# roljon/Steered-Mixture-of-Experts

Hardware: NVIDIA B200
Metric: pixel_kernel_evals_per_s_fwd_bwd (higher is better)
Workload: dtype f32

## Files before the change

### steered-mixture-of-experts_b200/csrc/forward.cu

```cuda
#include "smoe_common.cuh"
#include "fwd_records.cuh"

namespace smoe {

template <int D, int C>
__device__ __forceinline__ void parabola(const float* __restrict__ f, const float (&xs)[3], float& c, float& b) {
    using R = Rec<D, C>;
    c = f[R::OC];
#pragma unroll
    for (int l = 1; l < D; ++l) {
        float t = f[R::OL + l];
#pragma unroll
        for (int m = l; m < D; ++m) t = fmaf(f[R::OQ + ut(D, l, m)], xs[m], t);
        c = fmaf(t, xs[l], c);
    }
    b = f[R::OL + 0];
#pragma unroll
    for (int m = 1; m < D; ++m) b = fmaf(f[R::OQ + ut(D, 0, m)], xs[m], b);
}

struct FwdArgs {
    smoe_cfg cfg;
    smoe_batch b;
    const float* packed;
    const int32_t* indices;
    const int32_t* counts;
    const float* chunk_bounds;
    const float* lossw;
    const float* ax[3];
    float* rbuf;
    int32_t* argmax;
    uint8_t* infl;
    float* pix;
    float* tile_qmin;
    unsigned long long* pair_counts;
    int ntiles, nt1, nt2, max_chunks;
    float tau, ltau;
    float eps_cut;
};

#ifndef SMOE_FWD_UNROLL
#define SMOE_FWD_UNROLL 2
#endif
constexpr int kBodyUnroll = SMOE_FWD_UNROLL;
template <int D, int C, bool COUNT, bool AMAX>
__global__ void __launch_bounds__(kThreadsF, (D == 2) ? SMOE_FWD_CTAS_2D : 4) forward_kernel(const FwdArgs a) {
    using R = Rec<D, C>;
    constexpr int PK = pstride(D, C);
    constexpr int PPT = kPixPerThread;
    static_assert(kChunk == kThreadsF, "one kernel of a chunk per thread");
    extern __shared__ __align__(128) unsigned char smem_raw[];
    float* raw0 = reinterpret_cast<float*>(smem_raw);
    float* raw1 = raw0 + kChunk * PK;
    float* crec = raw1 + kChunk * PK;
    uint64_t* bar = reinterpret_cast<uint64_t*>(crec + kChunk * R::RC);
    float* red = reinterpret_cast<float*>(bar + 2);
    int* scratch = reinterpret_cast<int*>(red + 32);
    int* clist = scratch + 8;

    const int tid = threadIdx.x;
    const int K = a.counts[0];
    const int nchunks = (K + kChunk - 1) / kChunk;
    const int mode = a.cfg.dense_exec;
    const bool cull = mode == 0, skip = mode != 1;
    if (tid == 0) {
        mbar_init(&bar[0], 1);
        mbar_init(&bar[1], 1);
        fence_barrier_init();
    }
    __syncthreads();
    uint32_t phase0 = 0, phase1 = 0;
    int par = 0;
    unsigned cntA_vis = 0, cntA_ex = 0, cntB_vis = 0, cntB_ex = 0;

    auto issue = [&](int ci, int buf) {
        int nk = min(kChunk, K - ci * kChunk);
        uint32_t bytes = (uint32_t)nk * PK * 4u;
        fence_proxy_async();
        mbar_expect_tx(&bar[buf], bytes);
        tma_load_1d(buf ? raw1 : raw0, a.packed + (size_t)ci * kChunk * PK, bytes, &bar[buf]);
    };

    const int e1 = a.b.tile[1], e2 = a.b.tile[2];
    for (int tile = blockIdx.x; tile < a.ntiles; tile += gridDim.x) {
        int tt[3];
        tt[2] = tile % a.nt2;
        tt[1] = (tile / a.nt2) % a.nt1;
        tt[0] = tile / (a.nt2 * a.nt1);
        int lo[3], hi[3];
        float ctr[3], half[3];
#pragma unroll
        for (int i = 0; i < 3; ++i) {
            lo[i] = a.b.origin[i] + tt[i] * a.b.tile[i];
            hi[i] = min(lo[i] + a.b.tile[i], a.b.origin[i] + a.b.extent[i]) - 1;
            const float c0 = (i < D) ? a.ax[i][lo[i]] : 0.f, c1 = (i < D) ? a.ax[i][hi[i]] : 0.f;
            ctr[i] = 0.5f * (c0 + c1);
            half[i] = 0.5f * (c1 - c0) * 1.0001f + 1e-7f;
        }
        float x0[PPT], xs[3] = {0.f, 0.f, 0.f};
        unsigned okmask = 0;
        const int gbase12 = ((tid / e2) % e1 + lo[1]) * a.b.dims[2] + (tid % e2 + lo[2]);
        unsigned hmask = 0;
        {
            const int i2 = tid % e2, i1 = (tid / e2) % e1;
            const int g1 = lo[1] + i1, g2 = lo[2] + i2;
            auto in_halo = [&](int ax, int g) {
                const int o = a.b.origin[ax], e = o + a.b.extent[ax];
                return ax < D && ((o > 0 && g < o + a.b.halo) || (e < a.b.dims[ax] && g >= e - a.b.halo));
            };
            const bool h12 = a.b.halo > 0 && (in_halo(1, g1) || in_halo(2, g2));
            if (D > 1) xs[1] = a.ax[1][min(g1, hi[1])] - ctr[1];
            if (D > 2) xs[2] = a.ax[2][min(g2, hi[2])] - ctr[2];
#pragma unroll
            for (int p = 0; p < PPT; ++p) {
                const int j = p * kThreadsF + tid;
                const int i0 = j / (e2 * e1);
                const int g0 = lo[0] + i0;
                const bool ok = g0 <= hi[0] && g1 <= hi[1] && g2 <= hi[2];
                bool fed = ok;
                if (a.lossw && ok && a.lossw[g0 * a.b.dims[1] * a.b.dims[2] + gbase12] == SMOE_PIXEL_ABSENT) fed = false;
                if (fed) okmask |= 1u << p;
                if (a.b.halo > 0 && (h12 || in_halo(0, g0))) hmask |= 1u << p;
                x0[p] = a.ax[0][min(g0, hi[0])] - ctr[0];
            }
        }

        auto build_chunk_list = [&](float thr, int part) -> int {
            int n = 0;
            for (int base = 0; base < nchunks; base += kThreadsF) {
                const int ci = base + tid;
                bool need = false;
                if (ci < nchunks) {
                    const float* cb = a.chunk_bounds + (size_t)ci * kCB;
                    float d2 = 0.f, kd = 0.f;
#pragma unroll
                    for (int l = 0; l < D; ++l) {
                        const float mn = cb[l] - ctr[l], mx = cb[3 + l] - ctr[l];
                        const float gap = fmaxf(fmaxf(mn - half[l], -half[l] - mx), 0.f);
                        d2 = fmaf(gap, gap, d2);
                        kd = fmaxf(kd, cb[8 + l] * gap * gap);
                    }
                    const float lam = cb[6], drop = fmaxf(lam * d2, kd);
                    need = part != 1 || !(lam >= 0.f) || !(drop > kNearCut);
                    if (cull && need) need = !(lam >= 0.f) || !(cb[7] - drop < thr);
                }
                int tot;
                const int pos = cta_compact(need, scratch, par, &tot);
                if (need) clist[n + pos] = ci;
                n += tot;
            }
            __syncthreads();
            return n;
        };

        auto sweep = [&](int nlist, float thr, int part, auto&& body) {
            if (tid == 0 && nlist > 0) {
                issue(clist[0], 0);
                if (nlist > 1) issue(clist[1], 1);
            }
            for (int li = 0; li < nlist; ++li) {
                const int buf = li & 1;
                const int ci = clist[li];
                const int nk = min(kChunk, K - ci * kChunk);
                if (buf) { mbar_wait(&bar[1], phase1); phase1 ^= 1; } else { mbar_wait(&bar[0], phase0); phase0 ^= 1; }
                const float* raw = (buf ? raw1 : raw0) + tid * PK;
                bool need = tid < nk;
                float mu[D];
#pragma unroll
                for (int l = 0; l < D; ++l) mu[l] = need ? raw[off_mu(D, C) + l] - ctr[l] : 0.f;
                if (need && (cull || part != 0)) {
                    float d2 = 0.f, kd = 0.f;
#pragma unroll
                    for (int l = 0; l < D; ++l) {
                        const float gap = fmaxf(fabsf(mu[l]) - half[l], 0.f);
                        d2 = fmaf(gap, gap, d2);
                        kd = fmaxf(kd, raw[nparam(D, C) + 1 + l] * gap * gap);
                    }
                    const float lam = raw[nparam(D, C)], drop = fmaxf(lam * d2, kd);
                    if (part != 0) need = (part == 1) == (!(lam >= 0.f) || !(drop > kNearCut));
                    if (need && cull) need = !(lam >= 0.f) || !(raw[off_pi(D, C)] - drop < thr);
                }
                int nneed;
                const int pos = cta_compact(need, scratch, par, &nneed);
                if (need) transform_record<D, C>(raw, mu, ctr, a.indices[ci * kChunk + tid], crec + pos * R::RC);
                __syncthreads();
                if (tid == 0 && li + 2 < nlist) issue(clist[li + 2], buf);
#pragma unroll kBodyUnroll
                for (int kk = 0; kk < nneed; ++kk) body(crec + kk * R::RC);
            }
            __syncthreads();
        };

        float S[PPT];
        float cutA = -126.5f;
        if (a.eps_cut > 0.f && a.tile_qmin) {
            const float Lprev = a.tile_qmin[tile];
            cutA = fmaxf(cutA, Lprev - 2.0f - a.eps_cut);
            if (!(cutA == cutA)) cutA = -126.5f;
        }
        float Lneed = cutA > -126.5f ? cutA + a.eps_cut : -INFINITY;
        for (int attempt = 0; attempt < 2; ++attempt) {
#pragma unroll
            for (int p = 0; p < PPT; ++p) S[p] = 0.f;
            float skipA = cutA + 0.5f;
            auto bodyA = [&](const float* rec) {
                float f[4 * R::NG4];
                const float4* r4 = reinterpret_cast<const float4*>(rec);
#pragma unroll
                for (int j = 0; j < R::NG4; ++j) {
                    float4 v = r4[j];
                    f[4 * j] = v.x; f[4 * j + 1] = v.y; f[4 * j + 2] = v.z; f[4 * j + 3] = v.w;
                }
                float cq, bq;
                parabola<D, C>(f, xs, cq, bq);
                float q[PPT];
                float qmax = -INFINITY;
#pragma unroll
                for (int p = 0; p < PPT; ++p) {
                    q[p] = fmaf(fmaf(f[R::OQ], x0[p], bq), x0[p], cq);
                    qmax = fmaxf(qmax, q[p]);
                }
                if (COUNT) cntA_vis += PPT;
                if (__builtin_expect(!skip || __any_sync(0xffffffffu, qmax >= skipA), 0)) {
#pragma unroll
                    for (int p = 0; p < PPT; ++p) S[p] += ex2f(q[p]);
                    if (COUNT) cntA_ex += PPT;
                }
            };
            sweep(build_chunk_list(cutA, 1), cutA, 1, bodyA);
            {
                float Lt = INFINITY;
#pragma unroll
                for (int p = 0; p < PPT; ++p)
                    if ((okmask >> p) & 1u) Lt = fminf(Lt, log2f(S[p]));
                float Lmin = Lt;
#pragma unroll
                for (int o = 16; o > 0; o >>= 1) Lmin = fminf(Lmin, __shfl_xor_sync(0xffffffffu, Lmin, o));
                if ((tid & 31) == 0) red[tid >> 5] = Lmin;
                __syncthreads();
                Lmin = fminf(fminf(red[0], red[1]), fminf(red[2], red[3]));
                __syncthreads();
                float cut2 = cutA;
                if (skip && Lmin == Lmin) {
                    cut2 = fmaxf(cutA, Lmin - 25.5f);
                    if (Lt == Lt) skipA = fmaxf(skipA, Lt - 25.25f);
                }
                sweep(build_chunk_list(cut2, 2), cut2, 2, bodyA);
            }
            if (!(Lneed > -INFINITY)) break;
            float smin = INFINITY;
#pragma unroll
            for (int p = 0; p < PPT; ++p)
                if ((okmask >> p) & 1u) smin = fminf(smin, log2f(fmaxf(S[p], kSFloor)));
            const int bad = __syncthreads_or(smin < Lneed);
            if (!bad) break;
            cutA = -126.5f;
            Lneed = -INFINITY;
        }

        float qthr[PPT], r[PPT][C], bestw[PPT];
        int bestk[PPT];
        float qmin = INFINITY;
        unsigned live_mask = 0;
#pragma unroll
        for (int p = 0; p < PPT; ++p) {
            if (S[p] > kSFloor) live_mask |= 1u << p;
            float Sc = fmaxf(S[p], kSFloor);
            qthr[p] = ((okmask >> p) & 1u) ? log2f(Sc) : INFINITY;
            qmin = fminf(qmin, qthr[p]);
            bestw[p] = 0.f;
            bestk[p] = -1;
#pragma unroll
            for (int c = 0; c < C; ++c) r[p][c] = 0.f;
        }
#pragma unroll
        for (int o = 16; o > 0; o >>= 1) qmin = fminf(qmin, __shfl_xor_sync(0xffffffffu, qmin, o));
        if ((tid & 31) == 0) red[tid >> 5] = qmin;
        __syncthreads();
        qmin = fminf(fminf(red[0], red[1]), fminf(red[2], red[3]));
        __syncthreads();
        if (tid == 0 && a.tile_qmin) a.tile_qmin[tile] = qmin;
        {
            const float ltau = a.ltau;
            const float thrB = qmin + ltau - 0.01f;
            const int nlist = build_chunk_list(thrB, 0);
            sweep(nlist, thrB, 0, [&](const float* rec) {
                float f[R::RC];
                const float4* r4 = reinterpret_cast<const float4*>(rec);
#pragma unroll
                for (int j = 0; j < R::NG4; ++j) {
                    float4 v = r4[j];
                    f[4 * j] = v.x; f[4 * j + 1] = v.y; f[4 * j + 2] = v.z; f[4 * j + 3] = v.w;
                }
                float cq, bq;
                parabola<D, C>(f, xs, cq, bq);
                float q[PPT];
                bool any = false;
#pragma unroll
                for (int p = 0; p < PPT; ++p) {
                    q[p] = fmaf(fmaf(f[R::OQ], x0[p], bq), x0[p], cq) - qthr[p];
                    any |= (q[p] > ltau);
                }
                if (COUNT) cntB_vis += PPT;
                if (__builtin_expect(!skip || __any_sync(0xffffffffu, any), 0)) {
                    if (COUNT) cntB_ex += PPT;
#pragma unroll
                    for (int j = R::NG4; j < (R::OK + 4) / 4; ++j) {
                        float4 v = r4[j];
                        f[4 * j] = v.x; f[4 * j + 1] = v.y; f[4 * j + 2] = v.z; f[4 * j + 3] = v.w;
                    }
                    const int korig = __float_as_int(f[R::OK]);
                    float Eb[C];
#pragma unroll
                    for (int c = 0; c < C; ++c) {
                        Eb[c] = f[R::ONU + c];
#pragma unroll
                        for (int l = 1; l < D; ++l) Eb[c] = fmaf(f[R::OGA + l * C + c], xs[l], Eb[c]);
                    }
#pragma unroll
                    for (int p = 0; p < PPT; ++p) {
                        const float w = ex2f(q[p]);
                        const bool pass = q[p] > ltau;
                        const float wm = pass ? w : 0.f;
#pragma unroll
                        for (int c = 0; c < C; ++c) r[p][c] = fmaf(wm, fmaf(f[R::OGA + c], x0[p], Eb[c]), r[p][c]);
                        if (AMAX && pass && (w > bestw[p] || (w == bestw[p] && korig < bestk[p]))) { bestw[p] = w; bestk[p] = korig; }
                    }
                    if (any && a.infl) a.infl[korig] = 1;
                }
            });
        }

#pragma unroll
        for (int p = 0; p < PPT; ++p) {
            const int j = p * kThreadsF + tid;
            const bool inb = (okmask >> p) & 1u;
            const int gpix = (lo[0] + j / (e2 * e1)) * a.b.dims[1] * a.b.dims[2] + gbase12;
            const bool halo = ((hmask >> p) & 1u) || (a.lossw && inb && a.lossw[gpix] == SMOE_PIXEL_HALO);
            if (inb && !halo) {
#pragma unroll
                for (int c = 0; c < C; ++c) a.rbuf[(size_t)gpix * C + c] = r[p][c];
                if (AMAX) a.argmax[gpix] = bestk[p];
            }
            if (a.pix) {
                const int RLf = a.b.tile[D - 1];
                float* tp = a.pix + (size_t)tile * pix_stride(D, C, RLf);
                tp[PL_Z * SMOE_TPIX + j] = D == 1 ? x0[p] : xs[D - 1];
                tp[PL_QTHR * SMOE_TPIX + j] = inb ? qthr[p] : INFINITY;
                tp[PL_GR * SMOE_TPIX + j] = (inb && ((live_mask >> p) & 1u)) ? 1.f : 0.f;
                if (D > 1 && j % RLf == 0) {
                    const int row = j / RLf, nrows = SMOE_TPIX / RLf;
                    tp[pix_rowc_offset(C) + row] = x0[p];
#pragma unroll
                    for (int l = 1; l < D - 1; ++l) tp[pix_rowc_offset(C) + l * nrows + row] = xs[l];
                }
            }
        }
    }

    if (COUNT) {
        unsigned long long v[4] = {cntA_vis, cntA_ex, cntB_vis, cntB_ex};
#pragma unroll
        for (int q = 0; q < 4; ++q) {
#pragma unroll
            for (int o = 16; o > 0; o >>= 1) v[q] += __shfl_down_sync(0xffffffffu, v[q], o);
            if ((tid & 31) == 0) atomicAdd(&a.pair_counts[q], v[q]);
        }
    }

}

struct LossArgs {
    smoe_cfg cfg;
    smoe_batch b;
    const float* rbuf;
    const float* image;
    const uint8_t* image_u8;
    const float* lossw;
    float* res;
    float* pix;
    float* scalars;
    float* partials;
    int32_t* ticket;
    int ntiles, nt1, nt2, pix_tstride;
    float eps, q_scale, q_inv_scale;
};

template <int C>
__global__ void __launch_bounds__(256) loss_kernel(const LossArgs a) {
    const int tid = threadIdx.x;
    const int e1 = a.b.tile[1], e2 = a.b.tile[2];
    const int D = a.cfg.d;
    float lsum[C];
#pragma unroll
    for (int c = 0; c < C; ++c) lsum[c] = 0.f;
    float sqsum = 0.f;
    int nonfinite = 0;
    {
        int tt[3], lo[3], hi[3];
        tt[0] = blockIdx.y;
        tt[1] = a.nt2 == 1 ? (int)blockIdx.x : (int)blockIdx.x / a.nt2;
        tt[2] = a.nt2 == 1 ? 0 : (int)blockIdx.x % a.nt2;
        const int tile = (tt[0] * a.nt1 + tt[1]) * a.nt2 + tt[2];
#pragma unroll
        for (int i = 0; i < 3; ++i) {
            lo[i] = a.b.origin[i] + tt[i] * a.b.tile[i];
            hi[i] = min(lo[i] + a.b.tile[i], a.b.origin[i] + a.b.extent[i]) - 1;
        }
        auto in_halo = [&](int ax, int g) {
            const int o = a.b.origin[ax], e = o + a.b.extent[ax];
            return ax < D && ((o > 0 && g < o + a.b.halo) || (e < a.b.dims[ax] && g >= e - a.b.halo));
        };
        float* tp = a.pix ? a.pix + (size_t)tile * a.pix_tstride : nullptr;
        const int i2 = tid % e2, i1 = (tid / e2) % e1;
        const int g1 = lo[1] + i1, g2 = lo[2] + i2;
        const bool in12 = g1 <= hi[1] && g2 <= hi[2];
        const bool halo12 = a.b.halo > 0 && (in_halo(1, g1) || in_halo(2, g2));
        const int rows_per_pass = 256 / (e1 * e2);
        int g0 = lo[0] + tid / (e1 * e2);
        for (int j = tid; j < SMOE_TPIX; j += 256, g0 += rows_per_pass) {
            bool inb = in12 && g0 <= hi[0];
            const int gpix = inb ? (g0 * a.b.dims[1] + g1) * a.b.dims[2] + g2 : 0;
            const float lwv = (a.lossw && inb) ? a.lossw[gpix] : 1.f;
            if (lwv == SMOE_PIXEL_ABSENT) inb = false;
            const bool halo = lwv == SMOE_PIXEL_HALO || halo12 || (a.b.halo > 0 && in_halo(0, g0));
            float g[C], gr = 0.f;
#pragma unroll
            for (int c = 0; c < C; ++c) g[c] = 0.f;
            if (inb && !halo) {
#pragma unroll
                for (int c = 0; c < C; ++c) {
                    const size_t gi = (size_t)gpix * C + c;
                    const float rv = a.rbuf[gi];
                    if (!(fabsf(rv) <= 3.0e38f)) nonfinite = 1;
                    const float rc = fminf(fmaxf(rv, 0.f), 1.f);
                    const float kq = floorf(__fadd_rn(__fmul_rn(rc, a.q_inv_scale), 0.5f));
                    const float rq = __fmul_rn(kq, a.q_scale);
                    const float tgt = a.image_u8 ? __fdiv_rn((float)a.image_u8[gi], 255.0f) : a.image[gi];
                    const float diff = __fsub_rn(rq, tgt);
                    const float ad = fabsf(diff) - a.eps;
                    sqsum = fmaf(diff, diff, sqsum);
                    lsum[c] = a.lossw ? fmaf(ad * ad, lwv, lsum[c]) : fmaf(ad, ad, lsum[c]);
                    const float cw = a.cfg.use_yuv ? (c == 0 ? 0.75f : 0.125f) : (1.0f / C);
                    const float sgn = diff > 0.f ? 1.f : (diff < 0.f ? -1.f : 0.f);
                    const bool ste = (rv >= 0.f) && (rv <= 1.f);
                    g[c] = ste ? 2.f * ad * sgn * cw * a.b.inv_count : 0.f;
                    if (a.lossw) g[c] *= lwv;
                    gr = fmaf(g[c], rv, gr);
                    if (a.res) a.res[gi] = rq;
                }
            }
            if (tp) {
                const bool live = tp[PL_GR * SMOE_TPIX + j] != 0.f;
                tp[PL_GR * SMOE_TPIX + j] = live ? gr : 0.f;
#pragma unroll
                for (int c = 0; c < C; ++c) tp[(PL_G + c) * SMOE_TPIX + j] = g[c];
            }
        }
    }
    __shared__ float red[8][8];
    __shared__ float tree[256];
    __shared__ int s_last;
    const int nblk = gridDim.x * gridDim.y, bid = blockIdx.y * gridDim.x + blockIdx.x;
    float vals[8];
#pragma unroll
    for (int q = 0; q < 8; ++q) vals[q] = 0.f;
#pragma unroll
    for (int c = 0; c < C; ++c) vals[c] = lsum[c];
    vals[4] = sqsum;
    vals[5] = (float)nonfinite;
#pragma unroll
    for (int q = 0; q < 6; ++q)
#pragma unroll
        for (int o = 16; o > 0; o >>= 1) vals[q] += __shfl_down_sync(0xffffffffu, vals[q], o);
    if ((tid & 31) == 0)
#pragma unroll
        for (int q = 0; q < 8; ++q) red[tid >> 5][q] = vals[q];
    __syncthreads();
    if (tid < 8) {
        float s = 0.f;
        for (int wv = 0; wv < 8; ++wv) s += red[wv][tid];
        a.partials[(size_t)bid * 8 + tid] = s;
    }
    __threadfence();
    __syncthreads();
    if (tid == 0) s_last = (atomicAdd(a.ticket, 1) == nblk - 1);
    __syncthreads();
    if (s_last) {
        __threadfence();
        for (int q = 0; q < 6; ++q) {
            float s = 0.f;
            for (int bq = tid; bq < nblk; bq += 256) s += __ldcg(&a.partials[(size_t)bq * 8 + q]);
            tree[tid] = s;
            __syncthreads();
            for (int o = 128; o > 0; o >>= 1) {
                if (tid < o) tree[tid] += tree[tid + o];
                __syncthreads();
            }
            if (tid == 0) a.scalars[q] += tree[0];
            __syncthreads();
        }
        if (tid == 0) *a.ticket = 0;
    }
}

struct CotArgs {
    smoe_batch b;
    const float* rbuf;
    const float* grad_r;
    float* pix;
    int nt1, nt2, pix_tstride;
};

template <int C>
__global__ void __launch_bounds__(256) cotangent_kernel(const CotArgs a) {
    const int tid = threadIdx.x;
    const int e1 = a.b.tile[1], e2 = a.b.tile[2];
    int tt[3], lo[3], hi[3];
    tt[0] = blockIdx.y;
    tt[1] = a.nt2 == 1 ? (int)blockIdx.x : (int)blockIdx.x / a.nt2;
    tt[2] = a.nt2 == 1 ? 0 : (int)blockIdx.x % a.nt2;
    const int tile = (tt[0] * a.nt1 + tt[1]) * a.nt2 + tt[2];
#pragma unroll
    for (int i = 0; i < 3; ++i) {
        lo[i] = a.b.origin[i] + tt[i] * a.b.tile[i];
        hi[i] = min(lo[i] + a.b.tile[i], a.b.origin[i] + a.b.extent[i]) - 1;
    }
    float* tp = a.pix + (size_t)tile * a.pix_tstride;
    const int i2 = tid % e2, i1 = (tid / e2) % e1;
    const int g1 = lo[1] + i1, g2 = lo[2] + i2;
    const bool in12 = g1 <= hi[1] && g2 <= hi[2];
    const int rows_per_pass = 256 / (e1 * e2);
    int g0 = lo[0] + tid / (e1 * e2);
    for (int j = tid; j < SMOE_TPIX; j += 256, g0 += rows_per_pass) {
        const bool inb = in12 && g0 <= hi[0];
        const int gpix = inb ? (g0 * a.b.dims[1] + g1) * a.b.dims[2] + g2 : 0;
        float g[C], gr = 0.f;
#pragma unroll
        for (int c = 0; c < C; ++c) g[c] = 0.f;
        if (inb) {
#pragma unroll
            for (int c = 0; c < C; ++c) {
                const size_t gi = (size_t)gpix * C + c;
                g[c] = a.grad_r[gi];
                gr = fmaf(g[c], a.rbuf[gi], gr);
            }
        }
        const bool live = tp[PL_GR * SMOE_TPIX + j] != 0.f;
        tp[PL_GR * SMOE_TPIX + j] = live ? gr : 0.f;
#pragma unroll
        for (int c = 0; c < C; ++c) tp[(PL_G + c) * SMOE_TPIX + j] = g[c];
    }
}

template <int D, int C>
static size_t fwd_smem_bytes(int max_chunks) {
    return (size_t)(2 * kChunk * pstride(D, C) + kChunk * Rec<D, C>::RC) * 4 + 2 * 8 + 32 * 4 + 8 * 4 +
           (size_t)max_chunks * 4 + 64;
}

}

using namespace smoe;

extern "C" int smoe_forward(const smoe_cfg* cfg, const smoe_batch* batch, const float* packed, const int32_t* indices,
                            const int32_t* counts, const float* chunk_bounds, int K_cap, const float* loss_weights,
                            const float* ax0, const float* ax1, const float* ax2, float* rbuf, int32_t* argmax,
                            uint8_t* infl, float* pix, float* tile_qmin, unsigned long long* pair_counts, void* stream) {
    SMOE_REQUIRE(cfg && batch && packed && indices && counts && chunk_bounds && ax0 && ax1 && rbuf, "null argument");
    SMOE_REQUIRE(K_cap > 0, "K_cap must be positive");
    SMOE_REQUIRE(cfg->d == 2 || ax2, "ax2 required for d == 3");
    SMOE_REQUIRE(batch->tile[0] * batch->tile[1] * batch->tile[2] == SMOE_TPIX, "tile product must be SMOE_TPIX");
    SMOE_REQUIRE(kThreadsF % (batch->tile[1] * batch->tile[2]) == 0 && batch->tile[cfg->d - 1] % 4 == 0,
                 "tile[1]*tile[2] must divide 128 and the last tile extent must be a multiple of 4");
    SMOE_REQUIRE(!pix || tile_qmin, "tile_qmin is required with pix");
    SMOE_REQUIRE(batch->halo >= 0, "negative halo");
    SMOE_REQUIRE(cfg->eps_bits == 0 || (cfg->eps_bits >= 24 && cfg->eps_bits <= 126), "eps_bits must be 0 or in [24, 126]");
    SMOE_REQUIRE(cfg->eps_bits == 0 || cfg->dense_exec == 0, "eps_bits needs dense_exec == 0");
    for (int i = 0; i < 3; ++i)
        SMOE_REQUIRE(batch->extent[i] > 0 && batch->origin[i] >= 0 && batch->origin[i] + batch->extent[i] <= batch->dims[i],
                     "batch rectangle outside the image");
    SMOE_REQUIRE(cfg->d == 3 || (batch->dims[2] == 1 && batch->tile[2] == 1), "d == 2 needs dims[2] == tile[2] == 1");
    SMOE_REQUIRE((long long)batch->dims[0] * batch->dims[1] * batch->dims[2] < (1ll << 31), "more than 2^31 pixels");
    FwdArgs a;
    a.cfg = *cfg;
    a.b = *batch;
    a.packed = packed; a.indices = indices; a.counts = counts; a.chunk_bounds = chunk_bounds;
    a.lossw = loss_weights;
    a.ax[0] = ax0; a.ax[1] = ax1; a.ax[2] = ax2 ? ax2 : ax0;
    a.rbuf = rbuf; a.argmax = argmax; a.infl = infl; a.pix = pix; a.tile_qmin = tile_qmin;
    a.pair_counts = pair_counts;
    a.nt1 = (batch->extent[1] + batch->tile[1] - 1) / batch->tile[1];
    a.nt2 = (batch->extent[2] + batch->tile[2] - 1) / batch->tile[2];
    a.ntiles = smoe_num_tiles(batch);
    a.max_chunks = (K_cap + kChunk - 1) / kChunk;
    const float two_p = (float)(1 << cfg->precision);
    a.tau = 0.5f / two_p;
    a.ltau = -(float)(cfg->precision + 1);
    a.eps_cut = (float)cfg->eps_bits;
    int dev = 0, sms = 0;
    cudaGetDevice(&dev);
    cudaDeviceGetAttribute(&sms, cudaDevAttrMultiProcessorCount, dev);
    const int per_sm = cfg->d == 2 ? SMOE_FWD_CTAS_2D : 4;
    int grid = a.ntiles < per_sm * sms ? a.ntiles : per_sm * sms;
    cudaStream_t st = (cudaStream_t)stream;
#define LAUNCH(D, C, CNT, AM)                                                                                       \
    {                                                                                                               \
        size_t sm = fwd_smem_bytes<D, C>(a.max_chunks);                                                             \
        SMOE_REQUIRE(sm <= 200 * 1024, "too many kernel chunks for the shared-memory chunk list");                  \
        cudaFuncSetAttribute(forward_kernel<D, C, CNT, AM>, cudaFuncAttributeMaxDynamicSharedMemorySize, (int)sm);  \
        forward_kernel<D, C, CNT, AM><<<grid, kThreadsF, sm, st>>>(a);                                              \
    }
#define CALL(D, C)                                                               \
    if (pair_counts) { if (argmax) LAUNCH(D, C, true, true) else LAUNCH(D, C, true, false) } \
    else { if (argmax) LAUNCH(D, C, false, true) else LAUNCH(D, C, false, false) }
    SMOE_DISPATCH_DC(cfg->d, cfg->C, CALL)
#undef CALL
#undef LAUNCH
    return check_launch("smoe_forward");
}

extern "C" int smoe_loss_partials(const smoe_batch* batch) {
    return batch ? smoe_num_tiles(batch) : 0;
}

extern "C" int smoe_loss(const smoe_cfg* cfg, const smoe_batch* batch, const float* rbuf, const float* image,
                         const uint8_t* image_u8, const float* loss_weights, float* res, float* pix, float* scalars,
                         float* partials, int32_t* ticket, void* stream) {
    SMOE_REQUIRE(cfg && batch && rbuf && scalars && partials && ticket, "null argument");
    SMOE_REQUIRE((image != nullptr) != (image_u8 != nullptr), "exactly one of image / image_u8");
    SMOE_REQUIRE(batch->tile[0] * batch->tile[1] * batch->tile[2] == SMOE_TPIX, "tile product must be SMOE_TPIX");
    SMOE_REQUIRE(cfg->C == 1 || cfg->C == 3, "1 or 3 channels");
    SMOE_REQUIRE(256 % (batch->tile[1] * batch->tile[2]) == 0, "tile[1]*tile[2] must divide 256");
    LossArgs a;
    a.cfg = *cfg;
    a.b = *batch;
    a.rbuf = rbuf; a.image = image; a.image_u8 = image_u8; a.lossw = loss_weights; a.res = res; a.pix = pix;
    a.scalars = scalars; a.partials = partials; a.ticket = ticket;
    a.nt1 = (batch->extent[1] + batch->tile[1] - 1) / batch->tile[1];
    a.nt2 = (batch->extent[2] + batch->tile[2] - 1) / batch->tile[2];
    a.ntiles = smoe_num_tiles(batch);
    a.pix_tstride = pix_stride(cfg->d, cfg->C, batch->tile[cfg->d - 1]);
    const float two_p = (float)(1 << cfg->precision);
    a.eps = cfg->margin / two_p;
    a.q_scale = 1.0f / (two_p - 1.0f);
    a.q_inv_scale = 1.0f / a.q_scale;
    const int nt0 = a.ntiles / (a.nt1 * a.nt2);
    SMOE_REQUIRE(nt0 <= 65535, "too many tiles along the first axis");
    const dim3 grid(a.nt1 * a.nt2, nt0);
    if (cfg->C == 1) loss_kernel<1><<<grid, 256, 0, (cudaStream_t)stream>>>(a);
    else loss_kernel<3><<<grid, 256, 0, (cudaStream_t)stream>>>(a);
    return check_launch("smoe_loss");
}

extern "C" int smoe_cotangent(const smoe_cfg* cfg, const smoe_batch* batch, const float* rbuf, const float* grad_r,
                              float* pix, void* stream) {
    SMOE_REQUIRE(cfg && batch && rbuf && grad_r && pix, "null argument");
    SMOE_REQUIRE(batch->tile[0] * batch->tile[1] * batch->tile[2] == SMOE_TPIX, "tile product must be SMOE_TPIX");
    SMOE_REQUIRE(batch->halo == 0, "halo must be 0: the cotangent covers the whole batch rectangle");
    SMOE_REQUIRE((cfg->d == 2 || cfg->d == 3) && (cfg->C == 1 || cfg->C == 3), "d in {2, 3} and 1 or 3 channels");
    SMOE_REQUIRE(256 % (batch->tile[1] * batch->tile[2]) == 0, "tile[1]*tile[2] must divide 256");
    CotArgs a;
    a.b = *batch;
    a.rbuf = rbuf; a.grad_r = grad_r; a.pix = pix;
    a.nt1 = (batch->extent[1] + batch->tile[1] - 1) / batch->tile[1];
    a.nt2 = (batch->extent[2] + batch->tile[2] - 1) / batch->tile[2];
    a.pix_tstride = pix_stride(cfg->d, cfg->C, batch->tile[cfg->d - 1]);
    const int nt0 = smoe_num_tiles(batch) / (a.nt1 * a.nt2);
    SMOE_REQUIRE(nt0 <= 65535, "too many tiles along the first axis");
    const dim3 grid(a.nt1 * a.nt2, nt0);
    if (cfg->C == 1) cotangent_kernel<1><<<grid, 256, 0, (cudaStream_t)stream>>>(a);
    else cotangent_kernel<3><<<grid, 256, 0, (cudaStream_t)stream>>>(a);
    return check_launch("smoe_cotangent");
}
```

Before: 82860 billion.

## Cache transformed kernel records in shared memory across forward passes

Transformed kernel records from the pass-A sweeps are kept in a larger shared-memory cache, sized from the device's per-SM shared-memory budget. When pass-A culling covers the pass-B threshold, pass B reads the cached records instead of re-TMA-loading chunks and re-transforming them. The cached records are filtered and merged into global index order with a binary-search merge so results keep the same order. Per-chunk bound tests are computed once per tile instead of on every list build. The cost is much larger shared memory per CTA, which may lower occupancy, plus extra bookkeeping, a fallback path on cache overflow or a miss, and an optional stats instrumentation path.

```diff
diff --git a/steered-mixture-of-experts_b200/csrc/forward.cu b/steered-mixture-of-experts_b200/csrc/forward.cu
--- a/steered-mixture-of-experts_b200/csrc/forward.cu
+++ b/steered-mixture-of-experts_b200/csrc/forward.cu
@@ -35,6 +35,7 @@
     float* tile_qmin;
     unsigned long long* pair_counts;
     int ntiles, nt1, nt2, max_chunks;
+    int cache_cap;
     float tau, ltau;
     float eps_cut;
 };
@@ -43,20 +44,43 @@
 #define SMOE_FWD_UNROLL 2
 #endif
 constexpr int kBodyUnroll = SMOE_FWD_UNROLL;
+#ifndef SMOE_FWD_CACHE_MAX
+#define SMOE_FWD_CACHE_MAX 1024
+#endif
+#ifdef SMOE_FWD_STATS
+constexpr int kStatCols = 10, kStatTiles = 1 << 16;
+__device__ int g_fwd_stats[kStatTiles * kStatCols];
+#endif
+
+template <int D, int C>
+__host__ __device__ constexpr size_t fwd_smem_fixed(int max_chunks) {
+    return (size_t)2 * kChunk * pstride(D, C) * 4 + 2 * 8 + 32 * 4 + 8 * 4 + (size_t)max_chunks * 9 + 64;
+}
+template <int D, int C>
+__host__ __device__ constexpr size_t fwd_smem_per_rec() { return (size_t)Rec<D, C>::RC * 4 + 4 + 4 + 2 + 2; }
+
 template <int D, int C, bool COUNT, bool AMAX>
 __global__ void __launch_bounds__(kThreadsF, (D == 2) ? SMOE_FWD_CTAS_2D : 4) forward_kernel(const FwdArgs a) {
     using R = Rec<D, C>;
     constexpr int PK = pstride(D, C);
     constexpr int PPT = kPixPerThread;
     static_assert(kChunk == kThreadsF, "one kernel of a chunk per thread");
+    const int cap = a.cache_cap;
     extern __shared__ __align__(128) unsigned char smem_raw[];
     float* raw0 = reinterpret_cast<float*>(smem_raw);
     float* raw1 = raw0 + kChunk * PK;
     float* crec = raw1 + kChunk * PK;
-    uint64_t* bar = reinterpret_cast<uint64_t*>(crec + kChunk * R::RC);
+    uint64_t* bar = reinterpret_cast<uint64_t*>(crec + (size_t)cap * R::RC);
     float* red = reinterpret_cast<float*>(bar + 2);
+    int* tstate = reinterpret_cast<int*>(red + 8);
     int* scratch = reinterpret_cast<int*>(red + 32);
     int* clist = scratch + 8;
+    float* cbv = reinterpret_cast<float*>(clist + a.max_chunks);
+    int* cpos = reinterpret_cast<int*>(cbv + a.max_chunks);
+    float* cval = reinterpret_cast<float*>(cpos + cap);
+    unsigned short* ord1 = reinterpret_cast<unsigned short*>(cval + cap);
+    unsigned short* ord2 = ord1 + cap;
+    unsigned char* cnear = reinterpret_cast<unsigned char*>(ord2 + cap);
 
     const int tid = threadIdx.x;
     const int K = a.counts[0];
@@ -71,7 +95,14 @@
     __syncthreads();
     uint32_t phase0 = 0, phase1 = 0;
     int par = 0;
-    unsigned cntA_vis = 0, cntA_ex = 0, cntB_vis = 0, cntB_ex = 0;
+    unsigned cntA_vis = 0, cntA_ex = 0, cntB_vis = 0, cntB_ex = 0, cnt_cached = 0;
+    auto cta_min = [&](float v) -> float {
+#pragma unroll
+        for (int o = 16; o > 0; o >>= 1) v = fminf(v, __shfl_xor_sync(0xffffffffu, v, o));
+        if ((tid & 31) == 0) red[tid >> 5] = v;
+        __syncthreads();
+        return fminf(fminf(red[0], red[1]), fminf(red[2], red[3]));
+    };
 
     auto issue = [&](int ci, int buf) {
         int nk = min(kChunk, K - ci * kChunk);
@@ -100,7 +131,6 @@
         float x0[PPT], xs[3] = {0.f, 0.f, 0.f};
         unsigned okmask = 0;
         const int gbase12 = ((tid / e2) % e1 + lo[1]) * a.b.dims[2] + (tid % e2 + lo[2]);
-        unsigned hmask = 0;
         {
             const int i2 = tid % e2, i1 = (tid / e2) % e1;
             const int g1 = lo[1] + i1, g2 = lo[2] + i2;
@@ -120,29 +150,34 @@
                 bool fed = ok;
                 if (a.lossw && ok && a.lossw[g0 * a.b.dims[1] * a.b.dims[2] + gbase12] == SMOE_PIXEL_ABSENT) fed = false;
                 if (fed) okmask |= 1u << p;
-                if (a.b.halo > 0 && (h12 || in_halo(0, g0))) hmask |= 1u << p;
+                if (a.b.halo > 0 && (h12 || in_halo(0, g0))) okmask |= 1u << (PPT + p);
                 x0[p] = a.ax[0][min(g0, hi[0])] - ctr[0];
             }
         }
 
+        for (int ci = tid; ci < nchunks; ci += kThreadsF) {
+            const float* cb = a.chunk_bounds + (size_t)ci * kCB;
+            float d2 = 0.f, kd = 0.f;
+#pragma unroll
+            for (int l = 0; l < D; ++l) {
+                const float mn = cb[l] - ctr[l], mx = cb[3 + l] - ctr[l];
+                const float gap = fmaxf(fmaxf(mn - half[l], -half[l] - mx), 0.f);
+                d2 = fmaf(gap, gap, d2);
+                kd = fmaxf(kd, cb[8 + l] * gap * gap);
+            }
+            const float lam = cb[6], drop = fmaxf(lam * d2, kd);
+            cnear[ci] = !(lam >= 0.f) || !(drop > kNearCut);
+            cbv[ci] = lam >= 0.f ? cb[7] - drop : __int_as_float(0x7fc00000);
+        }
+        __syncthreads();
         auto build_chunk_list = [&](float thr, int part) -> int {
             int n = 0;
             for (int base = 0; base < nchunks; base += kThreadsF) {
                 const int ci = base + tid;
                 bool need = false;
                 if (ci < nchunks) {
-                    const float* cb = a.chunk_bounds + (size_t)ci * kCB;
-                    float d2 = 0.f, kd = 0.f;
-#pragma unroll
-                    for (int l = 0; l < D; ++l) {
-                        const float mn = cb[l] - ctr[l], mx = cb[3 + l] - ctr[l];
-                        const float gap = fmaxf(fmaxf(mn - half[l], -half[l] - mx), 0.f);
-                        d2 = fmaf(gap, gap, d2);
-                        kd = fmaxf(kd, cb[8 + l] * gap * gap);
-                    }
-                    const float lam = cb[6], drop = fmaxf(lam * d2, kd);
-                    need = part != 1 || !(lam >= 0.f) || !(drop > kNearCut);
-                    if (cull && need) need = !(lam >= 0.f) || !(cb[7] - drop < thr);
+                    need = part != 1 || cnear[ci];
+                    if (cull && need) need = !(cbv[ci] < thr);
                 }
                 int tot;
                 const int pos = cta_compact(need, scratch, par, &tot);
@@ -153,7 +188,16 @@
             return n;
         };
 
-        auto sweep = [&](int nlist, float thr, int part, auto&& body) {
+        int ncache = 0;
+        bool cached = false;
+#ifdef SMOE_FWD_STATS
+        int st[kStatCols] = {};
+#endif
+
+        auto sweep = [&](int nlist, float thr, int part, float cut1, auto&& body) {
+#ifdef SMOE_FWD_STATS
+            st[part == 0 ? 2 : part - 1] += nlist;
+#endif
             if (tid == 0 && nlist > 0) {
                 issue(clist[0], 0);
                 if (nlist > 1) issue(clist[1], 1);
@@ -168,6 +212,7 @@
                 float mu[D];
 #pragma unroll
                 for (int l = 0; l < D; ++l) mu[l] = need ? raw[off_mu(D, C) + l] - ctr[l] : 0.f;
+                float bnd = 0.f;
                 if (need && (cull || part != 0)) {
                     float d2 = 0.f, kd = 0.f;
 #pragma unroll
@@ -177,16 +222,33 @@
                         kd = fmaxf(kd, raw[nparam(D, C) + 1 + l] * gap * gap);
                     }
                     const float lam = raw[nparam(D, C)], drop = fmaxf(lam * d2, kd);
-                    if (part != 0) need = (part == 1) == (!(lam >= 0.f) || !(drop > kNearCut));
-                    if (need && cull) need = !(lam >= 0.f) || !(raw[off_pi(D, C)] - drop < thr);
+                    const bool near = !(lam >= 0.f) || !(drop > kNearCut);
+                    if (part == 2 && near && !(cnear[ci] && !(cbv[ci] < cut1))) tstate[0] = 1;
+                    if (part != 0) need = (part == 1) == near;
+                    bnd = lam >= 0.f ? raw[off_pi(D, C)] - drop : __int_as_float(0x7fc00000);
+                    if (need && cull) need = !(bnd < thr);
                 }
                 int nneed;
                 const int pos = cta_compact(need, scratch, par, &nneed);
-                if (need) transform_record<D, C>(raw, mu, ctr, a.indices[ci * kChunk + tid], crec + pos * R::RC);
+                int base = 0;
+                if (part != 0 && cached) {
+                    if (ncache + nneed <= cap) base = ncache;
+                    else cached = false;
+                }
+                if (need) {
+                    transform_record<D, C>(raw, mu, ctr, a.indices[ci * kChunk + tid], crec + (base + pos) * R::RC);
+                    cpos[base + pos] = ci * kChunk + tid;
+                    cval[base + pos] = bnd;
+                }
+                if (cached && part != 0) ncache += nneed;
+#ifdef SMOE_FWD_STATS
+                st[part == 0 ? 5 : 2 + part] += nneed;
+#endif
                 __syncthreads();
                 if (tid == 0 && li + 2 < nlist) issue(clist[li + 2], buf);
+                const float* cr = crec + base * R::RC;
 #pragma unroll kBodyUnroll
-                for (int kk = 0; kk < nneed; ++kk) body(crec + kk * R::RC);
+                for (int kk = 0; kk < nneed; ++kk) body(cr + kk * R::RC);
             }
             __syncthreads();
         };
@@ -200,6 +262,12 @@
         }
         float Lneed = cutA > -126.5f ? cutA + a.eps_cut : -INFINITY;
         for (int attempt = 0; attempt < 2; ++attempt) {
+            ncache = 0;
+            cached = cull;
+            if (tid == 0) tstate[0] = 0;
+#ifdef SMOE_FWD_STATS
+            st[0] = st[1] = st[3] = st[4] = 0;
+#endif
 #pragma unroll
             for (int p = 0; p < PPT; ++p) S[p] = 0.f;
             float skipA = cutA + 0.5f;
@@ -227,25 +295,21 @@
                     if (COUNT) cntA_ex += PPT;
                 }
             };
-            sweep(build_chunk_list(cutA, 1), cutA, 1, bodyA);
+            sweep(build_chunk_list(cutA, 1), cutA, 1, cutA, bodyA);
+            if (tid == 0) tstate[1] = ncache;
             {
                 float Lt = INFINITY;
 #pragma unroll
                 for (int p = 0; p < PPT; ++p)
                     if ((okmask >> p) & 1u) Lt = fminf(Lt, log2f(S[p]));
-                float Lmin = Lt;
-#pragma unroll
-                for (int o = 16; o > 0; o >>= 1) Lmin = fminf(Lmin, __shfl_xor_sync(0xffffffffu, Lmin, o));
-                if ((tid & 31) == 0) red[tid >> 5] = Lmin;
-                __syncthreads();
-                Lmin = fminf(fminf(red[0], red[1]), fminf(red[2], red[3]));
-                __syncthreads();
+                const float Lmin = cta_min(Lt);
                 float cut2 = cutA;
                 if (skip && Lmin == Lmin) {
                     cut2 = fmaxf(cutA, Lmin - 25.5f);
                     if (Lt == Lt) skipA = fmaxf(skipA, Lt - 25.25f);
                 }
-                sweep(build_chunk_list(cut2, 2), cut2, 2, bodyA);
+                if (tid == 0) tstate[2] = __float_as_int(cut2);
+                sweep(build_chunk_list(cut2, 2), cut2, 2, cutA, bodyA);
             }
             if (!(Lneed > -INFINITY)) break;
             float smin = INFINITY;
@@ -261,10 +325,9 @@
         float qthr[PPT], r[PPT][C], bestw[PPT];
         int bestk[PPT];
         float qmin = INFINITY;
-        unsigned live_mask = 0;
 #pragma unroll
         for (int p = 0; p < PPT; ++p) {
-            if (S[p] > kSFloor) live_mask |= 1u << p;
+            if (S[p] > kSFloor) okmask |= 1u << (2 * PPT + p);
             float Sc = fmaxf(S[p], kSFloor);
             qthr[p] = ((okmask >> p) & 1u) ? log2f(Sc) : INFINITY;
             qmin = fminf(qmin, qthr[p]);
@@ -273,18 +336,12 @@
 #pragma unroll
             for (int c = 0; c < C; ++c) r[p][c] = 0.f;
         }
-#pragma unroll
-        for (int o = 16; o > 0; o >>= 1) qmin = fminf(qmin, __shfl_xor_sync(0xffffffffu, qmin, o));
-        if ((tid & 31) == 0) red[tid >> 5] = qmin;
-        __syncthreads();
-        qmin = fminf(fminf(red[0], red[1]), fminf(red[2], red[3]));
-        __syncthreads();
+        qmin = cta_min(qmin);
         if (tid == 0 && a.tile_qmin) a.tile_qmin[tile] = qmin;
         {
             const float ltau = a.ltau;
             const float thrB = qmin + ltau - 0.01f;
-            const int nlist = build_chunk_list(thrB, 0);
-            sweep(nlist, thrB, 0, [&](const float* rec) {
+            auto bodyB = [&](const float* rec) {
                 float f[R::RC];
                 const float4* r4 = reinterpret_cast<const float4*>(rec);
 #pragma unroll
@@ -328,7 +385,60 @@
                     }
                     if (any && a.infl) a.infl[korig] = 1;
                 }
-            });
+            };
+            const bool miss = tstate[0] != 0;
+            const int n1 = tstate[1];
+            const float cut2 = __int_as_float(tstate[2]);
+            if (cached && !miss && thrB >= cut2) {
+                if (COUNT && tid == 0) ++cnt_cached;
+#ifdef SMOE_FWD_STATS
+                st[2] = build_chunk_list(thrB, 0);
+                st[7] = 1;
+#endif
+                int m = 0, m1 = 0;
+                for (int run = 0; run < 2; ++run) {
+                    const int rb = run ? n1 : 0, re = run ? ncache : n1;
+                    for (int b = rb; b < re; b += kThreadsF) {
+                        const int e = b + tid;
+                        bool need = false;
+                        if (e < re) need = !(cbv[cpos[e] / kChunk] < thrB) && !(cval[e] < thrB);
+                        int tot;
+                        const int pos = cta_compact(need, scratch, par, &tot);
+                        if (need) ord1[m + pos] = (unsigned short)e;
+                        m += tot;
+                    }
+                    if (run == 0) m1 = m;
+                }
+                __syncthreads();
+                for (int t = tid; t < m; t += kThreadsF) {
+                    const int e = ord1[t], key = cpos[e];
+                    int first = t < m1 ? m1 : 0, count = t < m1 ? m - m1 : m1;
+                    const int o0 = first;
+                    while (count > 0) {
+                        const int step = count >> 1;
+                        if (cpos[ord1[first + step]] < key) { first += step + 1; count -= step + 1; }
+                        else count = step;
+                    }
+                    ord2[(t < m1 ? t : t - m1) + (first - o0)] = (unsigned short)e;
+                }
+                __syncthreads();
+#ifdef SMOE_FWD_STATS
+                st[6] = m;
+#endif
+#pragma unroll 1
+                for (int kk = 0; kk < m; ++kk) bodyB(crec + ord2[kk] * R::RC);
+            } else {
+                sweep(build_chunk_list(thrB, 0), thrB, 0, thrB, bodyB);
+#ifdef SMOE_FWD_STATS
+                st[6] = st[5];
+                st[9] = (cull && !cached ? 1 : 0) | (miss ? 2 : 0) | (!(thrB >= cut2) ? 4 : 0);
+#endif
+            }
+#ifdef SMOE_FWD_STATS
+            st[8] = ncache;
+            if (tid == 0 && tile < kStatTiles)
+                for (int c = 0; c < kStatCols; ++c) g_fwd_stats[tile * kStatCols + c] = st[c];
+#endif
         }
 
 #pragma unroll
@@ -336,7 +446,7 @@
             const int j = p * kThreadsF + tid;
             const bool inb = (okmask >> p) & 1u;
             const int gpix = (lo[0] + j / (e2 * e1)) * a.b.dims[1] * a.b.dims[2] + gbase12;
-            const bool halo = ((hmask >> p) & 1u) || (a.lossw && inb && a.lossw[gpix] == SMOE_PIXEL_HALO);
+            const bool halo = ((okmask >> (PPT + p)) & 1u) || (a.lossw && inb && a.lossw[gpix] == SMOE_PIXEL_HALO);
             if (inb && !halo) {
 #pragma unroll
                 for (int c = 0; c < C; ++c) a.rbuf[(size_t)gpix * C + c] = r[p][c];
@@ -347,7 +457,7 @@
                 float* tp = a.pix + (size_t)tile * pix_stride(D, C, RLf);
                 tp[PL_Z * SMOE_TPIX + j] = D == 1 ? x0[p] : xs[D - 1];
                 tp[PL_QTHR * SMOE_TPIX + j] = inb ? qthr[p] : INFINITY;
-                tp[PL_GR * SMOE_TPIX + j] = (inb && ((live_mask >> p) & 1u)) ? 1.f : 0.f;
+                tp[PL_GR * SMOE_TPIX + j] = (inb && ((okmask >> (2 * PPT + p)) & 1u)) ? 1.f : 0.f;
                 if (D > 1 && j % RLf == 0) {
                     const int row = j / RLf, nrows = SMOE_TPIX / RLf;
                     tp[pix_rowc_offset(C) + row] = x0[p];
@@ -366,8 +476,8 @@
             for (int o = 16; o > 0; o >>= 1) v[q] += __shfl_down_sync(0xffffffffu, v[q], o);
             if ((tid & 31) == 0) atomicAdd(&a.pair_counts[q], v[q]);
         }
-    }
-
+        if (tid == 0 && cnt_cached) atomicAdd(&a.pair_counts[7], (unsigned long long)cnt_cached);
+    }
 }
 
 struct LossArgs {
@@ -554,9 +664,17 @@
 }
 
 template <int D, int C>
-static size_t fwd_smem_bytes(int max_chunks) {
-    return (size_t)(2 * kChunk * pstride(D, C) + kChunk * Rec<D, C>::RC) * 4 + 2 * 8 + 32 * 4 + 8 * 4 +
-           (size_t)max_chunks * 4 + 64;
+static int fwd_cache_cap(int max_chunks, int per_sm, int dev) {
+    int sm_per_sm = 0, reserved = 0;
+    cudaDeviceGetAttribute(&sm_per_sm, cudaDevAttrMaxSharedMemoryPerMultiprocessor, dev);
+    cudaDeviceGetAttribute(&reserved, cudaDevAttrReservedSharedMemoryPerBlock, dev);
+    const long long budget = (long long)sm_per_sm / per_sm - reserved - (long long)fwd_smem_fixed<D, C>(max_chunks);
+    const long long cap = budget / (long long)fwd_smem_per_rec<D, C>();
+    return (int)(cap < kChunk ? kChunk : (cap > SMOE_FWD_CACHE_MAX ? SMOE_FWD_CACHE_MAX : cap));
+}
+template <int D, int C>
+static size_t fwd_smem_bytes(int max_chunks, int cap) {
+    return fwd_smem_fixed<D, C>(max_chunks) + (size_t)cap * fwd_smem_per_rec<D, C>();
 }
 
 }
@@ -606,7 +724,8 @@
     cudaStream_t st = (cudaStream_t)stream;
 #define LAUNCH(D, C, CNT, AM)                                                                                       \
     {                                                                                                               \
-        size_t sm = fwd_smem_bytes<D, C>(a.max_chunks);                                                             \
+        a.cache_cap = fwd_cache_cap<D, C>(a.max_chunks, per_sm, dev);                                               \
+        size_t sm = fwd_smem_bytes<D, C>(a.max_chunks, a.cache_cap);                                                \
         SMOE_REQUIRE(sm <= 200 * 1024, "too many kernel chunks for the shared-memory chunk list");                  \
         cudaFuncSetAttribute(forward_kernel<D, C, CNT, AM>, cudaFuncAttributeMaxDynamicSharedMemorySize, (int)sm);  \
         forward_kernel<D, C, CNT, AM><<<grid, kThreadsF, sm, st>>>(a);                                              \
@@ -619,6 +738,15 @@
 #undef LAUNCH
     return check_launch("smoe_forward");
 }
+
+#ifdef SMOE_FWD_STATS
+extern "C" int smoe_fwd_stats(int* out, int ntiles) {
+    SMOE_REQUIRE(out && ntiles > 0 && ntiles <= kStatTiles, "bad arguments");
+    cudaDeviceSynchronize();
+    cudaMemcpyFromSymbol(out, g_fwd_stats, sizeof(int) * kStatCols * ntiles);
+    return check_launch("smoe_fwd_stats");
+}
+#endif
 
 extern "C" int smoe_loss_partials(const smoe_batch* batch) {
     return batch ? smoe_num_tiles(batch) : 0;
```

New measurement: 83350 billion, median of 6. About the same (+0.6%).
